# sizhe-li/neural-jacobian-field

Hardware: AMD Instinct MI355X
Metric: rendered rays/s (64 samples/ray, 256^2 image) (higher is better)
Workload: dtype f32 (v_mfma_f32_32x32x2_f32: exact fp32 products, fp32 accumulate -- the reference's arithmetic)

## Files before the change

### include/njf_hip.h

```cpp
#ifndef NJF_HIP_H
#define NJF_HIP_H

#include <stddef.h>
#include <stdint.h>

#ifdef __cplusplus
extern "C" {
#endif

#define NJF_ABI_VERSION 20
#define NJF_MAX_ACTION_DIM 10
#define NJF_HIDDEN 128
#define NJF_LATENT 512
#define NJF_PE_DIM 63
#define NJF_ZDIM 384

#define NJF_RESNET_CHUNKS 22
#define NJF_RESNET_CHUNKS_F16 12
#define NJF_CHUNK_FLOATS 8192
#define NJF_RESNET_W_FLOATS (NJF_RESNET_CHUNKS * NJF_CHUNK_FLOATS)
#define NJF_RESNET_B_FLOATS (10 * 128 + 32)
#define NJF_COLOR_W_FLOATS NJF_CHUNK_FLOATS
#define NJF_COLOR_B_FLOATS (64 + 32)
#define NJF_TRANSFORMER_CHUNKS 7
// ... 120 lines not shown
  float* jac_pe;
  int* foot_idx;
  float* foot_w;
  float* den_act;
  float* col_in;
  float* col_act;
  float* frame_partials;
  const float* trgt_rgb;
  const float* trgt_flow;
  unsigned* jac_mask;
  unsigned* den_mask;
  int dump_f16;
} NjfRenderOutputs;

int njf_render_forward(const float* origins, const float* directions, int rays_per_batch,
                       const NjfCameras* cams, const NjfFeatureMap* gmap, int gmap_offset_density,
                       int gmap_offset_jacobian, int jacobian_kind ,
                       const float* w_density, const float* b_density,
                       const float* w_color, const float* b_color,
                       const float* w_jacobian, const float* b_jacobian,
                       const float* bins, int samples, const NjfRenderOutputs* out, int precision, void* stream);

int njf_reduce_frame_partials(const float* partials, int groups, float* out4, void* stream);
int njf_assemble_frame(const float* packets, int world, int packet_floats, int batch, int rays_per_batch, float rgb_scale,
                       float flow_scale, float* frame, float* scalars6, void* stream);

int njf_points_forward(const float* xyz, const float* dirs, int points_per_batch, const NjfCameras* cams,
                       const NjfFeatureMap* gmap, int gmap_offset_density, int gmap_offset_jacobian, int mode,
                       int jacobian_kind , const float* w_density, const float* b_density, const float* w_color, const float* b_color,
                       const float* w_jacobian, const float* b_jacobian,
                       float* density, float* color, float* flow, float* jacobian, float* geo, float* features, int precision,
                       void* stream);

typedef struct NjfFieldGrid {
  float origin[3];
  float step[3];
  int dims[3];
} NjfFieldGrid;

int njf_field_points(const NjfFieldGrid* grid, int batch, const int* indices, const int* count, int capacity, float* xyz,
                     void* stream);

#define NJF_FIELD_SELECT_BLOCK 1024
int njf_field_select(const NjfFieldGrid* grid, const NjfCameras* cams, int batch, const float* values, float threshold,
                     const int* indices, const int* count, int capacity, int* out_indices, int* out_count, int out_capacity,
                     int* workspace, void* stream);
// ... 204 lines not shown
```

### neural-jacobian-field_amd/csrc/njf_device.h

```cpp
#pragma once
#include <hip/hip_runtime.h>
#include <stdint.h>

__device__ __forceinline__ float relu_bits(float x) { return __int_as_float(max(__float_as_int(x), 0)); }

typedef float f32x16 __attribute__((ext_vector_type(16)));
typedef float f32x4 __attribute__((ext_vector_type(4)));
typedef _Float16 f16x8 __attribute__((ext_vector_type(8)));
typedef _Float16 f16x16 __attribute__((ext_vector_type(16)));
typedef _Float16 f16x32 __attribute__((ext_vector_type(32)));
typedef int i32x8 __attribute__((ext_vector_type(8)));
typedef int i32x4 __attribute__((ext_vector_type(4)));
typedef int i32x2 __attribute__((ext_vector_type(2)));
typedef unsigned u32x6 __attribute__((ext_vector_type(6)));

#define PREC_F32 0
#define PREC_F16X2 1
#define PREC_F16F6 2
#define PREC_F16 3

#define NJF_WAVES 4
#define NJF_THREADS (NJF_WAVES * 64)
#define NJF_CHUNK 8192

#define NJF_STREAM_BUFFERS 2
#define LDS_CTR_FLOATS 0
#define LDS_W0 0
#define LDS_W1 NJF_CHUNK
#define LDS_BIAS (NJF_STREAM_BUFFERS * NJF_CHUNK)
#define LDS_BIAS_FLOATS 2752
#define LDS_BIAS_FLOATS_PROPOSAL 1344
#define LDS_SCRATCH_PER_WAVE 528
#define LDS_FLOATS_RENDER (LDS_BIAS + LDS_BIAS_FLOATS + LDS_CTR_FLOATS)
#define LDS_FLOATS_PROPOSAL (LDS_BIAS + LDS_BIAS_FLOATS_PROPOSAL + NJF_WAVES * LDS_SCRATCH_PER_WAVE + LDS_CTR_FLOATS)
#define LDS_SCRATCH_PROPOSAL (LDS_BIAS + LDS_BIAS_FLOATS_PROPOSAL)

extern __shared__ __attribute__((aligned(16))) float njf_lds[];

__device__ __forceinline__ float mfma_step(float a, float b, f32x16& c) {
  c = __builtin_amdgcn_mfma_f32_32x32x2f32(a, b, c, 0, 0, 0);
  return 0.f;
}

#ifdef NJF_STAMPS
#define NJF_STAMP_SLOTS 1024
#ifdef NJF_STAMPS_PROPOSAL
#define NJF_STAMP_BASE LDS_FLOATS_PROPOSAL
#define NJF_STAMP_LOGS_PROPOSAL true
#else
#define NJF_STAMP_BASE LDS_FLOATS_RENDER
#define NJF_STAMP_LOGS_PROPOSAL false
#endif
__device__ unsigned njf_stamp_out[NJF_STAMP_SLOTS];
#define NJF_STAMP_FIELD int stamp_i;
#define NJF_STAMP_INIT(st) (st).stamp_i = -1
#define NJF_STAMP(st, tag)                                                                                   \
  do {                                                                                                       \
    if ((st).stamp_i >= 0 && (st).stamp_i < NJF_STAMP_SLOTS) {                                               \
      njf_lds[NJF_STAMP_BASE + (st).stamp_i] =                                                               \
          __uint_as_float(((unsigned)(tag) << 24) | ((unsigned)__builtin_readcyclecounter() & 0xffffffu));   \
      (st).stamp_i += 1;                                                                                     \
    }                                                                                                        \
  } while (0)
#define NJF_STAMP_P(st, tag) do { if (NJF_STAMP_LOGS_PROPOSAL) NJF_STAMP(st, tag); } while (0)
#define NJF_STAMP_ARM(st, IS_PROPOSAL, wave)                                                                                \
  const bool njf_stamping = ((IS_PROPOSAL) == NJF_STAMP_LOGS_PROPOSAL) && blockIdx.x == gridDim.x / 2 + 3 && (wave) == 1; \
  if (njf_stamping) (st).stamp_i = 0;                                                                                     \
  NJF_STAMP(st, 9)
#define NJF_STAMP_FLUSH(st, tag, lane)                                                                       \
  do {                                                                                                       \
    NJF_STAMP(st, tag);                                                                                      \
    if (njf_stamping)                                                                                        \
      for (int i_ = (lane); i_ < NJF_STAMP_SLOTS; i_ += 64)                                                  \
        njf_stamp_out[i_] = i_ < (st).stamp_i ? __float_as_uint(njf_lds[NJF_STAMP_BASE + i_]) : 0u;          \
  } while (0)
#define NJF_STAMP_PIN(...) asm volatile("" : __VA_ARGS__)
#define NJF_STAMP_LDS_FLOATS NJF_STAMP_SLOTS
#else
#define NJF_STAMP_FIELD
#define NJF_STAMP_INIT(st) do {} while (0)
#define NJF_STAMP(st, tag) do {} while (0)
#define NJF_STAMP_P(st, tag) do {} while (0)
#define NJF_STAMP_ARM(st, IS_PROPOSAL, wave) do {} while (0)
#define NJF_STAMP_FLUSH(st, tag, lane) do {} while (0)
#define NJF_STAMP_PIN(...) do {} while (0)
#define NJF_STAMP_LDS_FLOATS 0
#endif

struct WeightStreamState {
  __amdgpu_buffer_rsrc_t rsrc;
  int per_pass;
  int total;
  int idx;
  int in_pass;
  int dma_voff;
  int dma_soff;
  float* dma_dst;
  int dma_next;
  NJF_STAMP_FIELD
};
template <int GAP_AT_, int GAP_>
struct WeightStreamT : WeightStreamState {
  static constexpr int GAP_AT = GAP_AT_, GAP = GAP_;
// ... 1248 lines not shown
```

### neural-jacobian-field_amd/csrc/njf_kernels.hip

```cpp
#include <hip/hip_runtime.h>
#include <math.h>
#include <stdint.h>

#include <atomic>
#include <type_traits>

#include "../../include/njf_hip.h"
#include "njf_device.h"

enum {
  NJF_OK = 0,
  NJF_E_NULL = -1,
  NJF_E_SHAPE = -2,
  NJF_E_ACTION_DIM = -3,
  NJF_E_SAMPLES = -4,
  NJF_E_DOUT = -5,
  NJF_E_MODE = -6,
  NJF_E_GMAP = -7,
  NJF_E_VALUE = -8,
};

extern "C" int njf_abi_version(void) { return NJF_ABI_VERSION; }
extern "C" int njf_rays_per_workgroup(void) { return NJF_WAVES; }

// ... 1009 lines not shown
  if (!k_inv || !c2w || !origins || !directions) return NJF_E_NULL;
  if (batch < 1 || rays < 1) return NJF_E_SHAPE;
  if (!coords && (height < 1 || width < 1 || (long long)height * width != rays)) return NJF_E_SHAPE;
  const int n = batch * rays;
  raygen_kernel<<<(n + 255) / 256, 256, 0, (hipStream_t)stream>>>(coords, height, width, k_inv, c2w, batch, rays, origins,
                                                                 directions, z);
  return launch_status();
}

template <int PREC>
constexpr int resnet_chunks() { return PREC == PREC_F16 ? NJF_RESNET_CHUNKS_F16 : NJF_RESNET_CHUNKS; }
template <int PREC>
constexpr int resnet_gap_at() { return PREC == PREC_F16 ? NJF_RESNET_CHUNKS_F16 : 0x7fffffff; }
template <int PREC>
constexpr int resnet_gap() { return PREC == PREC_F16 ? NJF_RESNET_CHUNKS - NJF_RESNET_CHUNKS_F16 : 0; }

struct RayCommon {
  const float* origins;
  const float* directions;
  int rays_per_batch;
  int total_rays;
  NjfCameras cams;
  NjfFeatureMap gmap;
};

__device__ __forceinline__ void load_bias_block(const float* __restrict__ src, int n, int dst_off) {
  for (int i = threadIdx.x; i < n; i += NJF_THREADS) njf_lds[LDS_BIAS + dst_off + i] = src[i];
}

__device__ __forceinline__ float alpha_of(float ds) {
  const float series = ds * fmaf(-0.5f * ds, fmaf(-(1.0f / 3.0f) * ds, fmaf(-0.25f * ds, fmaf(-0.2f, ds, 1.0f), 1.0f), 1.0f), 1.0f);
  return ds < 0.0625f ? series : 1.0f - expf(-ds);
}

__device__ __forceinline__ float tile_weights(float delta, float sigma, bool valid, int j, float& carry) {
  const float ds = (valid && delta > 0.f) ? delta * sigma : 0.f;
  const float incl = half_scan(ds, j);
  float excl = __shfl_up(incl, 1, 32);
  if (j == 0) excl = 0.f;
  excl += carry;
  carry += __shfl(incl, 31, 32);
  return alpha_of(ds) * expf(-excl);
}

__device__ __forceinline__ void pdf_resample_ray(float* __restrict__ sc, const float* __restrict__ bins_in, int s_in,
                                                 const float* __restrict__ u, int s_out, float* __restrict__ bins_out,
                                                 int lane, bool store) {
// ... 72 lines not shown
  if (d.act) act = d.act_f16 ? (float*)((_Float16*)d.act + pidx * 128 + 64 * hh) : d.act + pidx * 128 + 64 * hh;
  ActDump dump{act, d.pe + pidx * 64 + 32 * hh, points * 128, d.mask ? d.mask + pidx * 4 + 2 * hh : nullptr, d.act_f16 != 0};
  if (hh == 0 && d.foot_idx != nullptr) {
    Footprint f;
    point_footprint(g, f);
    int* fi = d.foot_idx + pidx * 4;
    fi[0] = tex0 + f.t00 / texel_stride;
    fi[1] = tex0 + f.t01 / texel_stride;
    fi[2] = tex0 + f.t10 / texel_stride;
    fi[3] = tex0 + f.t11 / texel_stride;
    float* fw = d.foot_w + pidx * 4;
    fw[0] = f.w00;
    fw[1] = f.w01;
    fw[2] = f.w10;
    fw[3] = f.w11;
  }
  return dump;
}

template <int PREC, bool DUMP = false>
__global__ void __launch_bounds__(NJF_THREADS, 2) proposal_kernel(ProposalArgs a) {
  const int tid = threadIdx.x;
  const int wave = __builtin_amdgcn_readfirstlane(tid >> 6);
  const int lane = tid & 63, j = lane & 31, hh = lane >> 5;
  const int wg = xcd_remap(blockIdx.x, gridDim.x);
  const int ray = wg * NJF_WAVES + wave;
  const bool ray_ok = ray < a.rc.total_rays;
  const int rayc = min(ray, a.rc.total_rays - 1);
  const int b = rayc / a.rc.rays_per_batch;

  load_bias_block(a.b_pack, NJF_RESNET_B_FLOATS, 0);
  const int tiles = (a.s_in + 31) >> 5;
  WeightStream st;
  stream_begin(st, a.w_pack, resnet_chunks<PREC>(), tiles, wave, lane);
  NJF_STAMP_ARM(st, true, wave);

  CamCtx cam;
  load_ctx(a.rc.cams.ctxt_w2c, a.rc.cams.ctxt_k, b, cam);
  const float near = a.rc.cams.z_near[b], far = a.rc.cams.z_far[b];
  const float ox = a.rc.origins[3 * (size_t)rayc], oy = a.rc.origins[3 * (size_t)rayc + 1],
              oz = a.rc.origins[3 * (size_t)rayc + 2];
  const float dx = a.rc.directions[3 * (size_t)rayc], dy = a.rc.directions[3 * (size_t)rayc + 1],
              dz = a.rc.directions[3 * (size_t)rayc + 2];
  const float* gz = map_at<PREC>(a.rc.gmap.data, (size_t)b * a.rc.gmap.height * a.rc.gmap.width * a.rc.gmap.stride + a.gmap_offset);
  const float* bins = a.bins_in + (a.bins_per_ray ? (size_t)rayc * (a.s_in + 1) : 0);
  float* sc = njf_lds + LDS_SCRATCH_PROPOSAL + wave * LDS_SCRATCH_PER_WAVE;
  const float* bias = njf_lds + LDS_BIAS;

  float carry = 0.f;
  for (int t = 0; t < tiles; ++t) {
    const int s = t * 32 + j;
    const bool valid = s < a.s_in;
    const int sc_i = min(s, a.s_in - 1);
    const float b0 = bins[sc_i], b1 = bins[sc_i + 1];
    const float start = b0 * far + (1.0f - b0) * near;
    const float end = b1 * far + (1.0f - b1) * near;
    const float se = start + end;
    const float px = ox + (dx * se) / 2.0f, py = oy + (dy * se) / 2.0f, pz = oz + (dz * se) / 2.0f;
    PointGeom g;
    point_geometry(cam, px, py, pz, a.rc.gmap.height, a.rc.gmap.width, a.rc.gmap.stride, 0u, g);
    NJF_STAMP_P(st, 10);
    f32x16 pe[2];
    positional_encoding(g.xc, g.yc, g.zc, hh, pe);
    f32x16 out[1];
    ActDump dump{nullptr, nullptr, 0};
    if (DUMP && valid && ray_ok)
      dump = point_dump(a.dump, (size_t)ray * a.s_in + s, (size_t)a.rc.total_rays * a.s_in, hh, g,
                        b * a.rc.gmap.height * a.rc.gmap.width, a.rc.gmap.stride);
    resnet_tile<PREC, DUMP>(st, bias, gz, g, pe, wave, lane, out, dump);
    NJF_STAMP_P(st, 14);
    const float pre = __shfl(out[0][0], j, 64);
    const float sigma = expf(pre - 1.0f);
    const float w = tile_weights(end - start, sigma, valid, j, carry);
    if (valid && hh == 0) {
      float wa = w;
      if (a.anneal != 1.0f) wa = powf(w, a.anneal);
      sc[s] = wa + 0.01f;
      if (ray_ok) {
        if (a.weights_out) a.weights_out[(size_t)ray * a.s_in + s] = w;
        if (a.density_out) a.density_out[(size_t)ray * a.s_in + s] = sigma;
      }
    }
  }
  NJF_STAMP_P(st, 13);
  __syncthreads();
  const float* u = a.u + (a.u_per_ray ? (size_t)rayc * (a.s_out + 1) : 0);
  pdf_resample_ray(sc, bins, a.s_in, u, a.s_out, a.bins_out + (size_t)rayc * (a.s_out + 1), lane, ray_ok);
  NJF_STAMP_FLUSH(st, 15, lane);
}

template <int PREC, int DUMP, int SHARE = 0, class ST>
__device__ __forceinline__ float density_stage(ST& st, const float* __restrict__ gz_d, const PointGeom& g, int wave,
                                               int lane, f32x16 (&geo)[1], ActDump dump, TileShareF16* share = nullptr) {
  const int j = lane & 31, hh = lane >> 5;
  f32x16 pe[2];
  positional_encoding(g.xc, g.yc, g.zc, hh, pe);
  if constexpr (SHARE != 0) {
    share_tile(pe, *share);
    resnet_tile<PREC, false, SHARE>(st, njf_lds + LDS_BIAS, gz_d, g, pe, wave, lane, geo, dump, share);
  } else {
    resnet_tile<PREC, DUMP == 2>(st, njf_lds + LDS_BIAS, gz_d, g, pe, wave, lane, geo, dump);
  }
  return expf(__shfl(geo[0][15], j, 64) - 1.0f);
}

template <int PREC, int DUMP, class ST>
__device__ __forceinline__ void color_stage(ST& st, const f32x16 (&geo)[1], float dirx, float diry, float dirz,
                                            int wave, int lane, float (&rgb)[3], ColorDump cdump) {
  const int j = lane & 31, hh = lane >> 5;
  asm volatile("" : "+v"(dirx), "+v"(diry), "+v"(dirz));
  float sh[16];
// ... 78 lines not shown
struct SamplePlace {
  float delta, tm, px, py, pz;
};
__device__ __forceinline__ void place_sample(float b0, float b1, float near, float far, float ox,
                                             float oy, float oz, float dx, float dy, float dz, SamplePlace& sp) {
  asm volatile("" : "+v"(b0), "+v"(b1));
  const float start = b0 * far + (1.0f - b0) * near;
  const float end = b1 * far + (1.0f - b1) * near;
  const float se = start + end;
  sp.delta = end - start;
  sp.tm = se / 2.0f;
  sp.px = ox + (dx * se) / 2.0f;
  sp.py = oy + (dy * se) / 2.0f;
  sp.pz = oz + (dz * se) / 2.0f;
}

template <int JKIND, int PREC, int DUMP = 0, bool AF = true, int PRECJ = PREC>
__global__ void __launch_bounds__(NJF_THREADS, 2) render_kernel(RenderArgs a) {
  constexpr bool WITH_J = JKIND != 0;
  constexpr int J_CHUNKS = JKIND == 1 ? resnet_chunks<PRECJ>() : (JKIND == 2 ? NJF_TRANSFORMER_CHUNKS : 0);
  constexpr int J_BIAS = JKIND == 1 ? NJF_RESNET_B_FLOATS : NJF_TRANSFORMER_B_FLOATS;
  const int tid = threadIdx.x;
  const int wave = __builtin_amdgcn_readfirstlane(tid >> 6);
  const int lane = tid & 63, j = lane & 31, hh = lane >> 5;
  const int wg = xcd_remap(blockIdx.x, gridDim.x);
  const int ray = wg * NJF_WAVES + wave;
  const bool ray_ok = ray < a.rc.total_rays;
  const int rayc = min(ray, a.rc.total_rays - 1);
  const int b = rayc / a.rc.rays_per_batch;
  const int S = a.samples;

  load_bias_block(a.b_d, NJF_RESNET_B_FLOATS, 0);
  load_bias_block(a.b_c, NJF_COLOR_B_FLOATS, NJF_RESNET_B_FLOATS);
  if (WITH_J) load_bias_block(a.b_j, J_BIAS, NJF_RESNET_B_FLOATS + NJF_COLOR_B_FLOATS);
  const int tiles = (S + 31) >> 5;
  WeightStreamT<resnet_gap_at<PREC>(), resnet_gap<PREC>()> st;
  stream_begin(st, a.w_all, resnet_chunks<PREC>() + 1 + J_CHUNKS, tiles, wave, lane);
  NJF_STAMP_ARM(st, false, wave);

  CamCtx cam;
  load_ctx(a.rc.cams.ctxt_w2c, a.rc.cams.ctxt_k, b, cam);
  const float near = a.rc.cams.z_near[b], far = a.rc.cams.z_far[b];
  const float ox = a.rc.origins[3 * (size_t)rayc], oy = a.rc.origins[3 * (size_t)rayc + 1],
              oz = a.rc.origins[3 * (size_t)rayc + 2];
  const float dx = a.rc.directions[3 * (size_t)rayc], dy = a.rc.directions[3 * (size_t)rayc + 1],
              dz = a.rc.directions[3 * (size_t)rayc + 2];
  const size_t gbase = (size_t)b * a.rc.gmap.height * a.rc.gmap.width * a.rc.gmap.stride;
  const float* gz_d = map_at<PREC>(a.rc.gmap.data, gbase + a.goff_d);
  const float* gz_j = map_at<PRECJ>(a.rc.gmap.data, gbase + a.goff_j);
  const float* bins = a.bins + (size_t)rayc * (S + 1);
  const int A = a.rc.cams.action_dim;
  const float* action = a.rc.cams.action ? a.rc.cams.action + (size_t)b * A : nullptr;

  float carry = 0.f;
  float acc_rgb[3] = {0.f, 0.f, 0.f}, acc_w = 0.f, acc_wt = 0.f;
  float acc_p[3] = {0.f, 0.f, 0.f}, acc_pw[3] = {0.f, 0.f, 0.f};
  float tmin = 3.0e38f, tmax = -3.0e38f;
  f32x16 acc_j = (f32x16)(0.f);
  const bool want_af = AF && WITH_J && a.out.action_features != nullptr;

  for (int t = 0; t < tiles; ++t) {
    const int s = t * 32 + j;
    const bool valid = s < S;
    const int sc_i = min(s, S - 1);
    const size_t si = (size_t)ray * S + s;
    const bool store = valid && ray_ok;
    const float bin0 = bins[sc_i], bin1 = bins[sc_i + 1];
    PointGeom g;
    {
// ... 73 lines not shown
        if (hh == 0 && a.out.sample_flow) {
          a.out.sample_flow[3 * si] = flow[0];
          a.out.sample_flow[3 * si + 1] = flow[1];
          a.out.sample_flow[3 * si + 2] = flow[2];
        }
        if (a.out.jacobian) {
#pragma unroll
          for (int r = 0; r < 16; ++r) {
            const int d = 16 * hh + r;
            if (d < 3 * A) a.out.jacobian[si * (3 * A) + d] = jac[0][r];
          }
        }
      }
    }
    if (valid) {
      SamplePlace sp;
      place_sample(bin0, bin1, near, far, ox, oy, oz, dx, dy, dz, sp);
      acc_pw[0] = fmaf(w, sp.px + flow[0], acc_pw[0]);
      acc_pw[1] = fmaf(w, sp.py + flow[1], acc_pw[1]);
      acc_pw[2] = fmaf(w, sp.pz + flow[2], acc_pw[2]);
    }
  }

  NJF_STAMP_FLUSH(st, 13, lane);
  acc_w = half_sum(acc_w);
  acc_wt = half_sum(acc_wt);
  tmin = half_min(tmin);
  tmax = half_max(tmax);
#pragma unroll
  for (int c = 0; c < 3; ++c) {
    acc_rgb[c] = half_sum(acc_rgb[c]);
    acc_p[c] = half_sum(acc_p[c]);
    acc_pw[c] = half_sum(acc_pw[c]);
  }
  if (want_af) {
#pragma unroll
    for (int r = 0; r < 16; ++r) acc_j[r] = half_sum(acc_j[r]);
    if (ray_ok && j == 0) {
#pragma unroll
      for (int r = 0; r < 16; ++r) {
        const int d = 16 * hh + r;
        if (d < 3 * A) a.out.action_features[(size_t)ray * (3 * A) + d] = acc_j[r];
      }
    }
  }
  float flow2d[2] = {0.f, 0.f};
  if (ray_ok && lane == 0) {
// ... 35 lines not shown
      flow2d[1] = uv[1][1] - uv[0][1];
      a.out.flow[2 * (size_t)ray] = flow2d[0];
      a.out.flow[2 * (size_t)ray + 1] = flow2d[1];
    }
  }
  if (a.out.frame_partials) {
    float se_rgb = 0.f, se_flow = 0.f;
    if (ray_ok && lane == 0) {
      if (a.out.trgt_rgb && a.out.rgb) {
#pragma unroll
        for (int c = 0; c < 3; ++c) {
          const float d = acc_rgb[c] - a.out.trgt_rgb[3 * (size_t)ray + c];
          se_rgb = fmaf(d, d, se_rgb);
        }
      }
      if (a.out.trgt_flow && a.out.flow && a.rc.cams.trgt_w2c && a.rc.cams.trgt_k) {
#pragma unroll
        for (int c = 0; c < 2; ++c) {
          const float d = flow2d[c] - a.out.trgt_flow[2 * (size_t)ray + c];
          se_flow = fmaf(d, d, se_flow);
        }
      }
    }
    __syncthreads();
    if (lane == 0) {
      njf_lds[4 * wave + 0] = ray_ok ? tmin : 3.0e38f;
      njf_lds[4 * wave + 1] = ray_ok ? tmax : -3.0e38f;
      njf_lds[4 * wave + 2] = se_rgb;
      njf_lds[4 * wave + 3] = se_flow;
    }
    __syncthreads();
    if (tid == 0) {
      float mn = njf_lds[0], mx = njf_lds[1], s0 = njf_lds[2], s1 = njf_lds[3];
#pragma unroll
      for (int w = 1; w < NJF_WAVES; ++w) {
        mn = fminf(mn, njf_lds[4 * w]);
        mx = fmaxf(mx, njf_lds[4 * w + 1]);
        s0 += njf_lds[4 * w + 2];
        s1 += njf_lds[4 * w + 3];
      }
      float* dst = a.out.frame_partials + 4 * (size_t)wg;
      dst[0] = mn;
      dst[1] = mx;
      dst[2] = s0;
      dst[3] = s1;
    }
  }
}

__global__ void __launch_bounds__(256) reduce_frame_partials_kernel(const float* __restrict__ partials, int groups,
                                                                    float* __restrict__ out4) {
  __shared__ float red[4][256];
  float mn = 3.0e38f, mx = -3.0e38f, s0 = 0.f, s1 = 0.f;
  for (int g = threadIdx.x; g < groups; g += 256) {
    const f32x4 v = *(const f32x4*)(partials + 4 * (size_t)g);
    mn = fminf(mn, v[0]);
    mx = fmaxf(mx, v[1]);
    s0 += v[2];
    s1 += v[3];
  }
  red[0][threadIdx.x] = mn;
  red[1][threadIdx.x] = mx;
  red[2][threadIdx.x] = s0;
  red[3][threadIdx.x] = s1;
  __syncthreads();
  for (int o = 128; o >= 1; o >>= 1) {
    if ((int)threadIdx.x < o) {
      red[0][threadIdx.x] = fminf(red[0][threadIdx.x], red[0][threadIdx.x + o]);
      red[1][threadIdx.x] = fmaxf(red[1][threadIdx.x], red[1][threadIdx.x + o]);
// ... 4068 lines not shown
  if (precision == NJF_PRECISION_F16X2) return f(std::integral_constant<int, PREC_F16X2>{});
  if (precision == NJF_PRECISION_F16F6) return f(std::integral_constant<int, PREC_F16F6>{});
  if (precision == NJF_PRECISION_F16) {
    if constexpr (TRAIN) return NJF_E_MODE;
    else return f(std::integral_constant<int, PREC_F16>{});
  }
  return f(std::integral_constant<int, PREC_F32>{});
#endif
}
template <bool TRAIN = false, typename F>
static int with_precisions(int precision, F&& f) {
  const int d = density_precision(precision), j = jacobian_precision(precision);
#ifdef NJF_DEV_ONLY_PREC
  return with_precision<TRAIN>(d, [&](auto P) { return f(P, P); });
#else
  if (d == j) return with_precision<TRAIN>(d, [&](auto P) { return f(P, P); });
  if (d == NJF_PRECISION_F16F6) return f(std::integral_constant<int, PREC_F16F6>{}, std::integral_constant<int, PREC_F16X2>{});
  return f(std::integral_constant<int, PREC_F16X2>{}, std::integral_constant<int, PREC_F16F6>{});
#endif
}
#define NJF_P decltype(P)::value
#define NJF_PJ decltype(PJ)::value

extern "C" int njf_proposal_forward(const float* origins, const float* directions, int rays_per_batch,
                                    const NjfCameras* cams, const NjfFeatureMap* gmap, int gmap_offset,
                                    const float* w_pack, const float* b_pack, const float* bins_in, int bins_per_ray,
                                    int s_in, const float* u, int u_per_ray, int s_out, float anneal, float* bins_out,
                                    float* weights_out, float* density_out, const NjfActivationDump* dump,
                                    int precision, void* stream) {
  int rc = check_common(origins, directions, rays_per_batch, cams, gmap);
  if (rc) return rc;
  if (!w_pack || !b_pack || !bins_in || !u || !bins_out) return NJF_E_NULL;
  if (s_in < 1 || s_in > 256 || s_out < 1) return NJF_E_SAMPLES;
  if (!valid_base_precision(precision)) return NJF_E_MODE;
  if ((rc = check_gmap(gmap, gmap_offset, NJF_ZDIM, precision))) return rc;
  ProposalArgs a;
  a.rc = RayCommon{origins, directions, rays_per_batch, rays_per_batch * cams->batch, *cams, *gmap};
  a.gmap_offset = gmap_offset;
  a.w_pack = w_pack;
  a.b_pack = b_pack;
  a.bins_in = bins_in;
  a.bins_per_ray = bins_per_ray;
  a.s_in = s_in;
  a.u = u;
  a.u_per_ray = u_per_ray;
  a.s_out = s_out;
  a.anneal = anneal;
  a.bins_out = bins_out;
  a.weights_out = weights_out;
  a.density_out = density_out;
  a.dump = NjfActivationDump{nullptr, nullptr, nullptr, nullptr, nullptr, 0};
  if (dump != nullptr && dump->act != nullptr) {
    if (!dump->pe || !dump->foot_idx || !dump->foot_w) return NJF_E_NULL;
    a.dump = *dump;
    return with_precision<true>(precision, [&](auto P) {
      return launch_fused(proposal_kernel<NJF_P, true>, a, a.rc.total_rays, (hipStream_t)stream, LDS_FLOATS_PROPOSAL);
    });
  }
  return with_precision(precision, [&](auto P) {
    return launch_fused(proposal_kernel<NJF_P>, a, a.rc.total_rays, (hipStream_t)stream, LDS_FLOATS_PROPOSAL);
  });
}

static int check_jacobian(int kind, const NjfCameras* cams, const NjfFeatureMap* gmap, int goff_j, const float* w_j,
                          const float* b_j, int precision) {
  if (kind == NJF_JACOBIAN_NONE) return NJF_OK;
  if (kind != NJF_JACOBIAN_MLP && kind != NJF_JACOBIAN_TRANSFORMER) return NJF_E_MODE;
  if (!w_j || !b_j) return NJF_E_NULL;
  const int max_a = kind == NJF_JACOBIAN_MLP ? NJF_MAX_ACTION_DIM : 8;
  if (cams->action_dim < 1 || cams->action_dim > max_a) return NJF_E_ACTION_DIM;
  return check_gmap(gmap, goff_j, kind == NJF_JACOBIAN_MLP ? NJF_ZDIM : NJF_QDIM, jacobian_precision(precision));
}

static int check_contiguous(const float* w_d, const float* w_c, const float* w_j, bool with_j) {
  if (w_c != w_d + NJF_RESNET_W_FLOATS) return NJF_E_SHAPE;
  if (with_j && w_j != w_c + NJF_COLOR_W_FLOATS) return NJF_E_SHAPE;
  return NJF_OK;
}

extern "C" int njf_render_forward(const float* origins, const float* directions, int rays_per_batch,
                                  const NjfCameras* cams, const NjfFeatureMap* gmap, int gmap_offset_density,
                                  int gmap_offset_jacobian, int jacobian_kind, const float* w_density,
                                  const float* b_density, const float* w_color, const float* b_color,
                                  const float* w_jacobian, const float* b_jacobian, const float* bins, int samples,
                                  const NjfRenderOutputs* out, int precision, void* stream) {
  int rc = check_common(origins, directions, rays_per_batch, cams, gmap);
  if (rc) return rc;
  if (!w_density || !b_density || !w_color || !b_color || !bins || !out) return NJF_E_NULL;
  if (samples < 1) return NJF_E_SAMPLES;
  if (!valid_precision(precision)) return NJF_E_MODE;
  if ((rc = check_gmap(gmap, gmap_offset_density, NJF_ZDIM, density_precision(precision)))) return rc;
  if ((rc = check_jacobian(jacobian_kind, cams, gmap, gmap_offset_jacobian, w_jacobian, b_jacobian, precision))) return rc;
  const bool with_j = jacobian_kind != NJF_JACOBIAN_NONE;
  if ((rc = check_contiguous(w_density, w_color, w_jacobian, with_j))) return rc;
  RenderArgs a;
  a.rc = RayCommon{origins, directions, rays_per_batch, rays_per_batch * cams->batch, *cams, *gmap};
  a.goff_d = gmap_offset_density;
  a.goff_j = with_j ? gmap_offset_jacobian : gmap_offset_density;
  a.w_all = w_density;
  a.b_d = b_density;
  a.b_c = b_color;
  a.b_j = b_jacobian;
  a.bins = bins;
  a.samples = samples;
  a.out = *out;
  hipStream_t s = (hipStream_t)stream;
  const int n = a.rc.total_rays;
  constexpr bool TRAIN_AF = true;
  const bool training_forward = out->jac_act != nullptr || out->jac_pe != nullptr || out->den_act != nullptr;
  if (!TRAIN_AF && training_forward && out->action_features != nullptr) return NJF_E_MODE;
  if (out->jac_act != nullptr || (out->jac_pe != nullptr && out->den_act == nullptr)) {
    if (jacobian_kind == NJF_JACOBIAN_NONE || out->den_act) return NJF_E_MODE;
    if (!out->jac_pe || !out->foot_idx || !out->foot_w) return NJF_E_NULL;
    if (jacobian_kind == NJF_JACOBIAN_MLP) {
      if (!out->jac_act) return NJF_E_NULL;
      return with_precisions<true>(precision, [&](auto P, auto PJ) { return launch_fused(render_kernel<1, NJF_P, 1, TRAIN_AF, NJF_PJ>, a, n, s); });
    }
    if (out->dump_f16 || out->jac_mask) return NJF_E_MODE;
    return with_precisions<true>(precision, [&](auto P, auto PJ) { return launch_fused(render_kernel<2, NJF_P, 1, TRAIN_AF, NJF_PJ>, a, n, s); });
  }
  if (out->den_act != nullptr) {
    if (!out->jac_pe || !out->foot_idx || !out->foot_w || !out->col_in || !out->col_act) return NJF_E_NULL;
    if (jacobian_kind == NJF_JACOBIAN_NONE)
      return with_precision<true>(density_precision(precision), [&](auto P) { return launch_fused(render_kernel<0, NJF_P, 2, TRAIN_AF>, a, n, s); });
    return with_precisions<true>(precision, [&](auto P, auto PJ) {
      if (jacobian_kind == NJF_JACOBIAN_MLP) return launch_fused(render_kernel<1, NJF_P, 2, TRAIN_AF, NJF_PJ>, a, n, s);
      return launch_fused(render_kernel<2, NJF_P, 2, TRAIN_AF, NJF_PJ>, a, n, s);
    });
  }
  const bool af = with_j && out->action_features != nullptr;
  if (jacobian_kind == NJF_JACOBIAN_NONE)
    return with_precision(density_precision(precision), [&](auto P) { return launch_fused(render_kernel<0, NJF_P, 0, false>, a, n, s); });
  return with_precisions(precision, [&](auto P, auto PJ) {
    if (jacobian_kind == NJF_JACOBIAN_MLP)
      return af ? launch_fused(render_kernel<1, NJF_P, 0, true, NJF_PJ>, a, n, s) : launch_fused(render_kernel<1, NJF_P, 0, false, NJF_PJ>, a, n, s);
    return af ? launch_fused(render_kernel<2, NJF_P, 0, true, NJF_PJ>, a, n, s) : launch_fused(render_kernel<2, NJF_P, 0, false, NJF_PJ>, a, n, s);
  });
}

static int make_decoder_args(const NjfCameras* cams, const NjfFeatureMap* gmap, int gmap_offset_density, int gmap_offset_jacobian,
                             int mode, int jacobian_kind, bool density_only, const float* w_density, const float* b_density,
                             const float* w_color, const float* b_color, const float* w_jacobian, const float* b_jacobian,
                             int precision, DecoderArgs& a) {
  if (!cams || !gmap || !w_density || !b_density) return NJF_E_NULL;
  if (!cams->ctxt_w2c || !cams->ctxt_k || !gmap->data) return NJF_E_NULL;
  if (cams->batch < 1) return NJF_E_SHAPE;
  if (mode != 0 && mode != 1) return NJF_E_MODE;
  if (!valid_precision(precision)) return NJF_E_MODE;
  if (gmap->height < 1 || gmap->width < 1) return NJF_E_SHAPE;
  int rc;
  if ((rc = check_gmap(gmap, gmap_offset_density, NJF_ZDIM, density_precision(precision)))) return rc;
  if ((long long)cams->batch * gmap->height * gmap->width * gmap->stride > 0xffffffffLL) return NJF_E_SHAPE;
  int kmode = 0;
// ... 995 lines not shown
```

### neural-jacobian-field_amd/hip.py

```python

from __future__ import annotations

import ctypes as C
import math
import os
from typing import Dict, Optional

import torch

_HERE = os.path.dirname(os.path.abspath(__file__))
LIB_PATH = os.environ.get("NJF_HIP_LIB", os.path.join(_HERE, "libnjf_hip.so"))

MAX_ACTION_DIM = 10
ZDIM = 384
RESNET_W_FLOATS = 22 * 8192
RESNET_B_FLOATS = 10 * 128 + 32
COLOR_W_FLOATS = 8192
COLOR_B_FLOATS = 96
TRANSFORMER_W_FLOATS = 7 * 8192
TRANSFORMER_B_FLOATS = 3 * 256 + 32
QDIM = 64
JACOBIAN_NONE, JACOBIAN_MLP, JACOBIAN_TRANSFORMER = 0, 1, 2
PRECISIONS = {"f32": 0, "f16x2": 1, "f16f6": 2, "f16": 3}
REDUCED_PRECISIONS = ("f16",)
# ... 120 lines not shown
    "njf_field_band_leaks": ([C.POINTER(FieldGrid), C.c_int, _vp, _vp, _vp, C.c_int, _vp, _vp], C.c_int),
    "njf_field_twists": ([_vp, _vp, _vp, _vp, _vp, C.c_int, C.c_int, _vp, _vp, C.c_int] + [_vp] * 15 + [C.c_longlong, C.c_int, _vp],
                         C.c_int),
    "njf_field_joints": ([C.POINTER(FieldGrid), C.c_int, _vp, _vp, _vp, C.c_int, _vp, _vp, C.c_int, _vp, _vp, _vp, _vp, C.c_int,
                          C.c_int, C.c_int, C.c_int] + [_vp] * 9 + [C.c_longlong, C.c_int, _vp], C.c_int),
    "njf_field_pose": ([_vp, _vp, C.c_int, _vp, _vp, _vp, _vp, C.c_int, _vp, _vp, _vp, C.c_int, _vp, _vp, _vp, _vp, _vp, _vp, C.c_int,
                        _vp, _vp, _vp, _vp, _vp, _vp, _vp, C.c_int, _vp, _vp, _vp, C.c_longlong, C.c_int, _vp], C.c_int),
    "njf_field_commands": ([_vp, _vp, C.c_int, _vp, _vp, _vp, _vp, C.c_int, _vp, _vp, _vp, C.c_int, _vp, _vp, _vp, _vp, _vp, _vp, _vp, _vp,
                            C.c_int, _vp, C.c_int, _vp, C.c_int, _vp, _vp, _vp, C.c_double, C.c_int, C.c_double] + [_vp] * 11 +
                           [C.c_longlong, C.c_int, _vp], C.c_int),
    "njf_field_commands_metric": ([_vp, _vp, C.c_int, _vp, _vp, _vp, _vp, C.c_int, _vp, _vp, _vp, C.c_int, _vp, _vp, _vp, _vp, _vp, _vp, _vp,
                                   _vp, C.c_int, _vp, _vp, C.c_int, C.c_int, _vp, C.c_int, _vp, _vp, _vp, C.c_double, C.c_int,
                                   C.c_double] + [_vp] * 11 + [C.c_longlong, C.c_int, _vp], C.c_int),
    "njf_field_nearest": ([_vp, _vp, C.c_int, C.c_int, _vp, _vp, _vp, C.c_int, C.c_int, C.c_int, C.POINTER(FieldGrid), C.c_double,
                           _vp, _vp, _vp, _vp, _vp, C.c_longlong, C.c_int, _vp], C.c_int),
    "njf_pack_resnetfc_backward": ([C.POINTER(ResnetFcWeights), _vp, C.c_int, _vp], C.c_int),
    "njf_resnetfc_backward": ([_vp, C.c_int, _vp, _vp, C.c_int, _vp, _vp, _vp, C.c_int, _vp, _vp, _vp], C.c_int),
    "njf_pack_transformer_backward": ([_vp, _vp, _vp, C.c_int, _vp, _vp, C.c_int, _vp], C.c_int),
    "njf_transformer_backward": ([_vp, _vp, C.c_int, C.c_int, C.c_int, _vp, _vp, _vp, _vp, _vp, _vp, C.c_int, _vp, C.c_int, _vp], C.c_int),
    "njf_scatter_footprint": ([_vp, C.c_int, C.c_longlong, _vp, _vp, C.c_int, C.c_int, C.c_int, C.c_int, _vp, _vp], C.c_int),
    "njf_bn_act": ([_vp, _vp, _vp, _vp, _vp, C.c_float, _vp, C.c_int, C.c_int, C.c_int, C.c_int, _vp, _vp], C.c_int),
    "njf_relu_backward": ([_vp, _vp, _vp, C.c_int, C.c_int, C.c_int, _vp, _vp, _vp], C.c_int),
    "njf_reduce_frame_partials": ([_vp, C.c_int, _vp, _vp], C.c_int),
    "njf_assemble_frame": ([_vp, C.c_int, C.c_int, C.c_int, C.c_int, C.c_float, C.c_float, _vp, _vp, _vp], C.c_int),
    "njf_composite_backward": ([_vp, _vp, _vp, _vp, _vp, _vp, _vp, C.c_int, C.c_int, _vp, _vp, _vp], C.c_int),
    "njf_alpha_weights": ([_vp, _vp, C.c_int, C.c_int, _vp, _vp], C.c_int),
    "njf_pdf_resample": ([_vp, _vp, C.c_int, C.c_int, _vp, C.c_int, C.c_int, C.c_float, C.c_int, _vp, _vp], C.c_int),
}

EXPORTED_SYMBOLS = tuple(_SIGNATURES)


def load_library() -> C.CDLL:
    global _lib
    if _lib is None:
        if not os.path.exists(LIB_PATH):
            raise RuntimeError(
                f"{LIB_PATH} not found: the HIP extension is not built (run `python -c 'import __graft_entry__ as g; "
                "g.build()'`).  There is no CPU fallback for the rendering hot path.")
        lib = C.CDLL(LIB_PATH)
        for name, (argtypes, restype) in _SIGNATURES.items():
            fn = getattr(lib, name)
            fn.argtypes = argtypes
            fn.restype = restype
        _lib = lib
    return _lib
# ... 1117 lines not shown
    partial = torch.empty(blocks, channels, dtype=torch.float32, device=upstream.device) if want_colsum else None
    _launch("njf_relu_backward", load_library().njf_relu_backward, _ptr(upstream, "upstream"), _ptr(act, "act"), _ptr(residual, "residual"), points,
                                            channels, RELU_BACKWARD_ROWS, _ptr(out, "out"), _ptr(partial, "partial"))
    return out, (partial.sum(0) if want_colsum else None)


def bn_act(x: torch.Tensor, bn: "torch.nn.BatchNorm2d", skip: Optional[torch.Tensor] = None, relu: bool = True) -> torch.Tensor:
    b, c, h, w = x.shape
    if skip is not None and (skip.shape != x.shape or not skip.is_contiguous() or skip.dtype != torch.float32):
        raise ValueError("njf_hip: bn_act skip must be a contiguous float32 tensor of x's shape")
    if not x.is_contiguous() or bn.running_mean is None or bn.weight is None or bn.weight.numel() != c:
        raise ValueError("njf_hip: bn_act needs a contiguous NCHW tensor and an affine BatchNorm2d with running statistics")
    _launch("njf_bn_act", load_library().njf_bn_act, _ptr(x, "x"), _ptr(bn.weight.detach(), "gamma"), _ptr(bn.bias.detach(), "beta"),
            _ptr(bn.running_mean, "running_mean"), _ptr(bn.running_var, "running_var"), float(bn.eps), _ptr(skip, "skip"), int(relu),
            b, c, h * w, _ptr(x, "out"))
    return x


def frame_partial_groups(total_rays: int) -> int:
    per = load_library().njf_rays_per_workgroup()
    return (total_rays + per - 1) // per


def reduce_frame_partials(partials: torch.Tensor, out4: torch.Tensor) -> None:
    _launch("njf_reduce_frame_partials", load_library().njf_reduce_frame_partials, _ptr(partials, "partials"),
            partials.shape[0], _ptr(out4, "out4"))


def assemble_frame(packets: torch.Tensor, batch: int, rays_per_batch: int, frame: torch.Tensor, scalars6: torch.Tensor,
                   rgb_scale: float = 0.0, flow_scale: float = 0.0) -> None:
    world, packet_floats = packets.shape
    if tuple(frame.shape) != (batch, rays_per_batch, 6) or scalars6.numel() != 6:
        raise ValueError("njf_hip: assemble_frame shape mismatch")
    _launch("njf_assemble_frame", load_library().njf_assemble_frame, _ptr(packets, "packets"), world, packet_floats, batch,
            rays_per_batch, float(rgb_scale), float(flow_scale), _ptr(frame, "frame"), _ptr(scalars6, "scalars6"))


def composite_backward(deltas, steps, sigma, color=None, g_weights=None, g_rgb=None, g_depth=None, want_color: bool = True):
    if deltas.dim() != 2:
        raise ValueError("njf_hip: composite_backward takes [rays, samples] fields")
    rays, samples = deltas.shape
    for name, t, shape in (("steps", steps, (rays, samples)), ("sigma", sigma, (rays, samples)), ("g_weights", g_weights, (rays, samples)),
                           ("color", color, (rays, samples, 3)), ("g_rgb", g_rgb, (rays, 3)), ("g_depth", g_depth, (rays,))):
        if t is not None and tuple(t.shape) != shape:
            raise ValueError(f"njf_hip: composite_backward: {name} has shape {tuple(t.shape)}, expected {shape}")
    g_sigma = torch.empty(rays, samples, dtype=torch.float32, device=deltas.device)
# ... 19 lines not shown
```

Before: 2.030 million.

## Let render and proposal workgroups loop over multiple ray groups

```diff
diff --git a/include/njf_hip.h b/include/njf_hip.h
--- a/include/njf_hip.h
+++ b/include/njf_hip.h
@@ -166,6 +166,9 @@
                        const float* bins, int samples, const NjfRenderOutputs* out, int precision, void* stream);
 
 int njf_reduce_frame_partials(const float* partials, int groups, float* out4, void* stream);
+
+int njf_set_ray_groups_per_workgroup(int g);
+int njf_ray_groups_auto(int groups, int compute_units);
 int njf_assemble_frame(const float* packets, int world, int packet_floats, int batch, int rays_per_batch, float rgb_scale,
                        float flow_scale, float* frame, float* scalars6, void* stream);
 
diff --git a/neural-jacobian-field_amd/csrc/njf_device.h b/neural-jacobian-field_amd/csrc/njf_device.h
--- a/neural-jacobian-field_amd/csrc/njf_device.h
+++ b/neural-jacobian-field_amd/csrc/njf_device.h
@@ -24,7 +24,7 @@
 #define NJF_CHUNK 8192
 
 #define NJF_STREAM_BUFFERS 2
-#define LDS_CTR_FLOATS 0
+#define LDS_CTR_FLOATS 16
 #define LDS_W0 0
 #define LDS_W1 NJF_CHUNK
 #define LDS_BIAS (NJF_STREAM_BUFFERS * NJF_CHUNK)
@@ -32,7 +32,8 @@
 #define LDS_BIAS_FLOATS_PROPOSAL 1344
 #define LDS_SCRATCH_PER_WAVE 528
 #define LDS_FLOATS_RENDER (LDS_BIAS + LDS_BIAS_FLOATS + LDS_CTR_FLOATS)
-#define LDS_FLOATS_PROPOSAL (LDS_BIAS + LDS_BIAS_FLOATS_PROPOSAL + NJF_WAVES * LDS_SCRATCH_PER_WAVE + LDS_CTR_FLOATS)
+#define LDS_FLOATS_PROPOSAL (LDS_BIAS + LDS_BIAS_FLOATS_PROPOSAL + NJF_WAVES * LDS_SCRATCH_PER_WAVE)
+#define LDS_PARTIALS (LDS_BIAS + LDS_BIAS_FLOATS)
 #define LDS_SCRATCH_PROPOSAL (LDS_BIAS + LDS_BIAS_FLOATS_PROPOSAL)
 
 extern __shared__ __attribute__((aligned(16))) float njf_lds[];
@@ -54,6 +55,7 @@
 __device__ unsigned njf_stamp_out[NJF_STAMP_SLOTS];
 #define NJF_STAMP_FIELD int stamp_i;
 #define NJF_STAMP_INIT(st) (st).stamp_i = -1
+#define NJF_STAMP_DISARM(st) (st).stamp_i = -1
 #define NJF_STAMP(st, tag)                                                                                   \
   do {                                                                                                       \
     if ((st).stamp_i >= 0 && (st).stamp_i < NJF_STAMP_SLOTS) {                                               \
@@ -79,6 +81,7 @@
 #else
 #define NJF_STAMP_FIELD
 #define NJF_STAMP_INIT(st) do {} while (0)
+#define NJF_STAMP_DISARM(st) do {} while (0)
 #define NJF_STAMP(st, tag) do {} while (0)
 #define NJF_STAMP_P(st, tag) do {} while (0)
 #define NJF_STAMP_ARM(st, IS_PROPOSAL, wave) do {} while (0)
diff --git a/neural-jacobian-field_amd/csrc/njf_kernels.hip b/neural-jacobian-field_amd/csrc/njf_kernels.hip
--- a/neural-jacobian-field_amd/csrc/njf_kernels.hip
+++ b/neural-jacobian-field_amd/csrc/njf_kernels.hip
@@ -1055,7 +1055,39 @@
   int total_rays;
   NjfCameras cams;
   NjfFeatureMap gmap;
+  int groups_per_wg;
 };
+
+template <bool SINGLE>
+__device__ __forceinline__ int ray_groups_of(const RayCommon& rc, int wg, int& first) {
+  if constexpr (SINGLE) {
+    first = wg;
+    return 1;
+  } else {
+    const int groups = (rc.total_rays + NJF_WAVES - 1) / NJF_WAVES;
+    first = wg * rc.groups_per_wg;
+    return min(rc.groups_per_wg, groups - first);
+  }
+}
+
+template <bool SINGLE>
+__device__ __forceinline__ float group_uniform(float x) {
+  if constexpr (SINGLE) return x;
+  else return __int_as_float(__builtin_amdgcn_readfirstlane(__float_as_int(x)));
+}
+template <bool SINGLE>
+__device__ __forceinline__ int group_lane(int lane) {
+  if constexpr (!SINGLE) asm volatile("" : "+v"(lane));
+  return lane;
+}
+template <bool SINGLE>
+__device__ __forceinline__ void load_group_ctx(const float* __restrict__ w2c, const float* __restrict__ k, int b, CamCtx& c) {
+  load_ctx(w2c, k, b, c);
+#pragma unroll
+  for (int i = 0; i < 12; ++i) c.m[i] = group_uniform<SINGLE>(c.m[i]);
+#pragma unroll
+  for (int i = 0; i < 9; ++i) c.k[i] = group_uniform<SINGLE>(c.k[i]);
+}
 
 __device__ __forceinline__ void load_bias_block(const float* __restrict__ src, int n, int dst_off) {
   for (int i = threadIdx.x; i < n; i += NJF_THREADS) njf_lds[LDS_BIAS + dst_off + i] = src[i];
@@ -1174,30 +1206,34 @@
 __global__ void __launch_bounds__(NJF_THREADS, 2) proposal_kernel(ProposalArgs a) {
   const int tid = threadIdx.x;
   const int wave = __builtin_amdgcn_readfirstlane(tid >> 6);
-  const int lane = tid & 63, j = lane & 31, hh = lane >> 5;
+  const int lane_wg = tid & 63;
   const int wg = xcd_remap(blockIdx.x, gridDim.x);
-  const int ray = wg * NJF_WAVES + wave;
+  int group0;
+  const int n_groups = ray_groups_of<DUMP>(a.rc, wg, group0);
+
+  load_bias_block(a.b_pack, NJF_RESNET_B_FLOATS, 0);
+  const int tiles = (a.s_in + 31) >> 5;
+  WeightStream st;
+  stream_begin(st, a.w_pack, resnet_chunks<PREC>(), tiles * n_groups, wave, lane_wg);
+  NJF_STAMP_ARM(st, true, wave);
+  float* sc = njf_lds + LDS_SCRATCH_PROPOSAL + wave * LDS_SCRATCH_PER_WAVE;
+  const float* bias = njf_lds + LDS_BIAS;
+
+  for (int gi = 0; gi < n_groups; ++gi) {
+  const int lane = group_lane<DUMP>(lane_wg), j = lane & 31, hh = lane >> 5;
+  const int ray = (group0 + gi) * NJF_WAVES + wave;
   const bool ray_ok = ray < a.rc.total_rays;
   const int rayc = min(ray, a.rc.total_rays - 1);
   const int b = rayc / a.rc.rays_per_batch;
-
-  load_bias_block(a.b_pack, NJF_RESNET_B_FLOATS, 0);
-  const int tiles = (a.s_in + 31) >> 5;
-  WeightStream st;
-  stream_begin(st, a.w_pack, resnet_chunks<PREC>(), tiles, wave, lane);
-  NJF_STAMP_ARM(st, true, wave);
-
   CamCtx cam;
-  load_ctx(a.rc.cams.ctxt_w2c, a.rc.cams.ctxt_k, b, cam);
-  const float near = a.rc.cams.z_near[b], far = a.rc.cams.z_far[b];
-  const float ox = a.rc.origins[3 * (size_t)rayc], oy = a.rc.origins[3 * (size_t)rayc + 1],
-              oz = a.rc.origins[3 * (size_t)rayc + 2];
-  const float dx = a.rc.directions[3 * (size_t)rayc], dy = a.rc.directions[3 * (size_t)rayc + 1],
-              dz = a.rc.directions[3 * (size_t)rayc + 2];
+  load_group_ctx<DUMP>(a.rc.cams.ctxt_w2c, a.rc.cams.ctxt_k, b, cam);
+  const float near = group_uniform<DUMP>(a.rc.cams.z_near[b]), far = group_uniform<DUMP>(a.rc.cams.z_far[b]);
+  const float ox = group_uniform<DUMP>(a.rc.origins[3 * (size_t)rayc]), oy = group_uniform<DUMP>(a.rc.origins[3 * (size_t)rayc + 1]),
+              oz = group_uniform<DUMP>(a.rc.origins[3 * (size_t)rayc + 2]);
+  const float dx = group_uniform<DUMP>(a.rc.directions[3 * (size_t)rayc]), dy = group_uniform<DUMP>(a.rc.directions[3 * (size_t)rayc + 1]),
+              dz = group_uniform<DUMP>(a.rc.directions[3 * (size_t)rayc + 2]);
   const float* gz = map_at<PREC>(a.rc.gmap.data, (size_t)b * a.rc.gmap.height * a.rc.gmap.width * a.rc.gmap.stride + a.gmap_offset);
   const float* bins = a.bins_in + (a.bins_per_ray ? (size_t)rayc * (a.s_in + 1) : 0);
-  float* sc = njf_lds + LDS_SCRATCH_PROPOSAL + wave * LDS_SCRATCH_PER_WAVE;
-  const float* bias = njf_lds + LDS_BIAS;
 
   float carry = 0.f;
   for (int t = 0; t < tiles; ++t) {
@@ -1238,7 +1274,11 @@
   __syncthreads();
   const float* u = a.u + (a.u_per_ray ? (size_t)rayc * (a.s_out + 1) : 0);
   pdf_resample_ray(sc, bins, a.s_in, u, a.s_out, a.bins_out + (size_t)rayc * (a.s_out + 1), lane, ray_ok);
-  NJF_STAMP_FLUSH(st, 15, lane);
+  if (gi == 0) {
+    NJF_STAMP_FLUSH(st, 15, lane);
+    NJF_STAMP_DISARM(st);
+  }
+  }
 }
 
 template <int PREC, int DUMP, int SHARE = 0, class ST>
@@ -1363,29 +1403,35 @@
   constexpr int J_BIAS = JKIND == 1 ? NJF_RESNET_B_FLOATS : NJF_TRANSFORMER_B_FLOATS;
   const int tid = threadIdx.x;
   const int wave = __builtin_amdgcn_readfirstlane(tid >> 6);
-  const int lane = tid & 63, j = lane & 31, hh = lane >> 5;
+  const int lane_wg = tid & 63;
   const int wg = xcd_remap(blockIdx.x, gridDim.x);
-  const int ray = wg * NJF_WAVES + wave;
-  const bool ray_ok = ray < a.rc.total_rays;
-  const int rayc = min(ray, a.rc.total_rays - 1);
-  const int b = rayc / a.rc.rays_per_batch;
+  int group0;
+  const int n_groups = ray_groups_of<DUMP != 0>(a.rc, wg, group0);
   const int S = a.samples;
 
   load_bias_block(a.b_d, NJF_RESNET_B_FLOATS, 0);
   load_bias_block(a.b_c, NJF_COLOR_B_FLOATS, NJF_RESNET_B_FLOATS);
   if (WITH_J) load_bias_block(a.b_j, J_BIAS, NJF_RESNET_B_FLOATS + NJF_COLOR_B_FLOATS);
   const int tiles = (S + 31) >> 5;
+  __builtin_assume(tiles >= 1);
   WeightStreamT<resnet_gap_at<PREC>(), resnet_gap<PREC>()> st;
-  stream_begin(st, a.w_all, resnet_chunks<PREC>() + 1 + J_CHUNKS, tiles, wave, lane);
+  stream_begin(st, a.w_all, resnet_chunks<PREC>() + 1 + J_CHUNKS, tiles * n_groups, wave, lane_wg);
   NJF_STAMP_ARM(st, false, wave);
 
+  for (int gi = 0; gi < n_groups; ++gi) {
+  const int lane = group_lane<DUMP != 0>(lane_wg), j = lane & 31, hh = lane >> 5;
+  const int group = group0 + gi;
+  const int ray = group * NJF_WAVES + wave;
+  const bool ray_ok = ray < a.rc.total_rays;
+  const int rayc = min(ray, a.rc.total_rays - 1);
+  const int b = rayc / a.rc.rays_per_batch;
   CamCtx cam;
-  load_ctx(a.rc.cams.ctxt_w2c, a.rc.cams.ctxt_k, b, cam);
-  const float near = a.rc.cams.z_near[b], far = a.rc.cams.z_far[b];
-  const float ox = a.rc.origins[3 * (size_t)rayc], oy = a.rc.origins[3 * (size_t)rayc + 1],
-              oz = a.rc.origins[3 * (size_t)rayc + 2];
-  const float dx = a.rc.directions[3 * (size_t)rayc], dy = a.rc.directions[3 * (size_t)rayc + 1],
-              dz = a.rc.directions[3 * (size_t)rayc + 2];
+  load_group_ctx<DUMP != 0>(a.rc.cams.ctxt_w2c, a.rc.cams.ctxt_k, b, cam);
+  const float near = group_uniform<DUMP != 0>(a.rc.cams.z_near[b]), far = group_uniform<DUMP != 0>(a.rc.cams.z_far[b]);
+  const float ox = group_uniform<DUMP != 0>(a.rc.origins[3 * (size_t)rayc]), oy = group_uniform<DUMP != 0>(a.rc.origins[3 * (size_t)rayc + 1]),
+              oz = group_uniform<DUMP != 0>(a.rc.origins[3 * (size_t)rayc + 2]);
+  const float dx = group_uniform<DUMP != 0>(a.rc.directions[3 * (size_t)rayc]), dy = group_uniform<DUMP != 0>(a.rc.directions[3 * (size_t)rayc + 1]),
+              dz = group_uniform<DUMP != 0>(a.rc.directions[3 * (size_t)rayc + 2]);
   const size_t gbase = (size_t)b * a.rc.gmap.height * a.rc.gmap.width * a.rc.gmap.stride;
   const float* gz_d = map_at<PREC>(a.rc.gmap.data, gbase + a.goff_d);
   const float* gz_j = map_at<PRECJ>(a.rc.gmap.data, gbase + a.goff_j);
@@ -1505,7 +1551,10 @@
     }
   }
 
-  NJF_STAMP_FLUSH(st, 13, lane);
+  if (gi == 0) {
+    NJF_STAMP_FLUSH(st, 13, lane);
+    NJF_STAMP_DISARM(st);
+  }
   acc_w = half_sum(acc_w);
   acc_wt = half_sum(acc_wt);
   tmin = half_min(tmin);
@@ -1587,29 +1636,30 @@
         }
       }
     }
-    __syncthreads();
+    float* part = njf_lds + LDS_PARTIALS;
     if (lane == 0) {
-      njf_lds[4 * wave + 0] = ray_ok ? tmin : 3.0e38f;
-      njf_lds[4 * wave + 1] = ray_ok ? tmax : -3.0e38f;
-      njf_lds[4 * wave + 2] = se_rgb;
-      njf_lds[4 * wave + 3] = se_flow;
+      part[4 * wave + 0] = ray_ok ? tmin : 3.0e38f;
+      part[4 * wave + 1] = ray_ok ? tmax : -3.0e38f;
+      part[4 * wave + 2] = se_rgb;
+      part[4 * wave + 3] = se_flow;
     }
     __syncthreads();
     if (tid == 0) {
-      float mn = njf_lds[0], mx = njf_lds[1], s0 = njf_lds[2], s1 = njf_lds[3];
+      float mn = part[0], mx = part[1], s0 = part[2], s1 = part[3];
 #pragma unroll
       for (int w = 1; w < NJF_WAVES; ++w) {
-        mn = fminf(mn, njf_lds[4 * w]);
-        mx = fmaxf(mx, njf_lds[4 * w + 1]);
-        s0 += njf_lds[4 * w + 2];
-        s1 += njf_lds[4 * w + 3];
-      }
-      float* dst = a.out.frame_partials + 4 * (size_t)wg;
+        mn = fminf(mn, part[4 * w]);
+        mx = fmaxf(mx, part[4 * w + 1]);
+        s0 += part[4 * w + 2];
+        s1 += part[4 * w + 3];
+      }
+      float* dst = a.out.frame_partials + 4 * (size_t)group;
       dst[0] = mn;
       dst[1] = mx;
       dst[2] = s0;
       dst[3] = s1;
     }
+  }
   }
 }
 
@@ -5724,6 +5774,51 @@
 #define NJF_P decltype(P)::value
 #define NJF_PJ decltype(PJ)::value
 
+#define NJF_RAY_GROUPS_LIMIT 64
+#define RAY_GROUPS_AUTO_MAX 1
+#define RAY_GROUPS_ROUNDS_MIN 4
+static std::atomic<int> g_ray_groups{0};
+static std::atomic<int> g_compute_units[16];
+
+extern "C" int njf_ray_groups_auto(int groups, int compute_units) {
+  if (groups < 1 || compute_units < 1) return NJF_E_VALUE;
+  const long long floor_wgs = (long long)RAY_GROUPS_ROUNDS_MIN * 2 * compute_units;
+  int g = 1;
+  while (2 * g <= RAY_GROUPS_AUTO_MAX && (groups + 2 * g - 1) / (2 * g) >= floor_wgs) g *= 2;
+  return g;
+}
+
+extern "C" int njf_set_ray_groups_per_workgroup(int g) {
+  if (g < 0 || g > NJF_RAY_GROUPS_LIMIT) return NJF_E_VALUE;
+  return g_ray_groups.exchange(g, std::memory_order_acq_rel);
+}
+
+static int device_compute_units() {
+  int dev = 0;
+  if (hipGetDevice(&dev) != hipSuccess) return 0;
+  const bool cached = dev >= 0 && dev < 16;
+  int n = cached ? g_compute_units[dev].load(std::memory_order_acquire) : 0;
+  if (n == 0) {
+    if (hipDeviceGetAttribute(&n, hipDeviceAttributeMultiprocessorCount, dev) != hipSuccess || n < 1) return 0;
+    if (cached) g_compute_units[dev].store(n, std::memory_order_release);
+  }
+  return n;
+}
+
+static int ray_work_items(RayCommon& rc, bool single) {
+  const int groups = (rc.total_rays + NJF_WAVES - 1) / NJF_WAVES;
+  int g = 1;
+  if (!single) {
+    g = g_ray_groups.load(std::memory_order_acquire);
+    if (g == 0) {
+      const int cus = device_compute_units();
+      g = cus > 0 ? njf_ray_groups_auto(groups, cus) : 1;
+    }
+  }
+  rc.groups_per_wg = g;
+  return (groups + g - 1) / g * NJF_WAVES;
+}
+
 extern "C" int njf_proposal_forward(const float* origins, const float* directions, int rays_per_batch,
                                     const NjfCameras* cams, const NjfFeatureMap* gmap, int gmap_offset,
                                     const float* w_pack, const float* b_pack, const float* bins_in, int bins_per_ray,
@@ -5756,11 +5851,12 @@
     if (!dump->pe || !dump->foot_idx || !dump->foot_w) return NJF_E_NULL;
     a.dump = *dump;
     return with_precision<true>(precision, [&](auto P) {
-      return launch_fused(proposal_kernel<NJF_P, true>, a, a.rc.total_rays, (hipStream_t)stream, LDS_FLOATS_PROPOSAL);
+      return launch_fused(proposal_kernel<NJF_P, true>, a, ray_work_items(a.rc, true), (hipStream_t)stream, LDS_FLOATS_PROPOSAL);
     });
   }
+  const int n = ray_work_items(a.rc, false);
   return with_precision(precision, [&](auto P) {
-    return launch_fused(proposal_kernel<NJF_P>, a, a.rc.total_rays, (hipStream_t)stream, LDS_FLOATS_PROPOSAL);
+    return launch_fused(proposal_kernel<NJF_P>, a, n, (hipStream_t)stream, LDS_FLOATS_PROPOSAL);
   });
 }
 
@@ -5807,7 +5903,7 @@
   a.samples = samples;
   a.out = *out;
   hipStream_t s = (hipStream_t)stream;
-  const int n = a.rc.total_rays;
+  int n = ray_work_items(a.rc, true);
   constexpr bool TRAIN_AF = true;
   const bool training_forward = out->jac_act != nullptr || out->jac_pe != nullptr || out->den_act != nullptr;
   if (!TRAIN_AF && training_forward && out->action_features != nullptr) return NJF_E_MODE;
@@ -5831,6 +5927,7 @@
     });
   }
   const bool af = with_j && out->action_features != nullptr;
+  n = ray_work_items(a.rc, false);
   if (jacobian_kind == NJF_JACOBIAN_NONE)
     return with_precision(density_precision(precision), [&](auto P) { return launch_fused(render_kernel<0, NJF_P, 0, false>, a, n, s); });
   return with_precisions(precision, [&](auto P, auto PJ) {
diff --git a/neural-jacobian-field_amd/hip.py b/neural-jacobian-field_amd/hip.py
--- a/neural-jacobian-field_amd/hip.py
+++ b/neural-jacobian-field_amd/hip.py
@@ -166,6 +166,8 @@
     "njf_bn_act": ([_vp, _vp, _vp, _vp, _vp, C.c_float, _vp, C.c_int, C.c_int, C.c_int, C.c_int, _vp, _vp], C.c_int),
     "njf_relu_backward": ([_vp, _vp, _vp, C.c_int, C.c_int, C.c_int, _vp, _vp, _vp], C.c_int),
     "njf_reduce_frame_partials": ([_vp, C.c_int, _vp, _vp], C.c_int),
+    "njf_set_ray_groups_per_workgroup": ([C.c_int], C.c_int),
+    "njf_ray_groups_auto": ([C.c_int, C.c_int], C.c_int),
     "njf_assemble_frame": ([_vp, C.c_int, C.c_int, C.c_int, C.c_int, C.c_float, C.c_float, _vp, _vp, _vp], C.c_int),
     "njf_composite_backward": ([_vp, _vp, _vp, _vp, _vp, _vp, _vp, C.c_int, C.c_int, _vp, _vp, _vp], C.c_int),
     "njf_alpha_weights": ([_vp, _vp, C.c_int, C.c_int, _vp, _vp], C.c_int),
@@ -1329,6 +1331,18 @@
     return (total_rays + per - 1) // per
 
 
+def set_ray_groups_per_workgroup(g: int) -> int:
+    prev = load_library().njf_set_ray_groups_per_workgroup(int(g))
+    _check(min(prev, 0))
+    return prev
+
+
+def ray_groups_auto(groups: int, compute_units: int) -> int:
+    g = load_library().njf_ray_groups_auto(int(groups), int(compute_units))
+    _check(min(g, 0))
+    return g
+
+
 def reduce_frame_partials(partials: torch.Tensor, out4: torch.Tensor) -> None:
     _launch("njf_reduce_frame_partials", load_library().njf_reduce_frame_partials, _ptr(partials, "partials"),
             partials.shape[0], _ptr(out4, "out4"))
```

After: 2.021 million. Within noise of the previous version (-0.4%).
